# quasirandom/decoupled-kg

Measured on AMD Instinct MI355X. Metric: KG-evals/s (q=1, n_train=256, n_disc=1024, 16×128 MC) at 1/2/4/8 MI355X, higher is better.
Workload: dtype f64

## Files before the change

### decoupled-kg_amd/csrc/dkg_common.h

```cpp
#pragma once

#include <hip/hip_runtime.h>
#include <stdint.h>

#include <map>
#include <mutex>
#include <utility>

#include "dkg.h"

namespace dkg {

inline void raise_lds_limit(const void* kernel, size_t lds) {
  if (lds <= 65536) return;
  static std::mutex mu;
  static std::map<std::pair<const void*, int>, size_t> done;
  int dev = 0;
  (void)hipGetDevice(&dev);
  std::lock_guard<std::mutex> lock(mu);
  size_t& cur = done[{kernel, dev}];
  if (cur >= lds) return;
  if (hipFuncSetAttribute(kernel, hipFuncAttributeMaxDynamicSharedMemorySize, (int)lds) == hipSuccess) cur = lds;
}

// ... 195 lines not shown
__device__ __forceinline__ double norm_pdf(double c) { return 0.3989422804014327 * exp(-0.5 * c * c); }
__device__ __forceinline__ double norm_cdf(double c) { return 0.5 * erfc(-0.7071067811865476 * c); }

__device__ __forceinline__ double scaled_r2(const double* __restrict__ xa, const double* __restrict__ xb,
                                            const double* __restrict__ il, int d) {
  double acc = 0.0;
  for (int k = 0; k < d; ++k) {
    const double t = (xa[k] - xb[k]) * il[k];
    acc = fma(t, t, acc);
  }
  return acc;
}

template <int DM>
__device__ __forceinline__ double scaled_r2_dm(const double* __restrict__ xa, const double* __restrict__ xb,
                                               const double* __restrict__ il, int d) {
  double acc = 0.0;
#pragma unroll
  for (int k = 0; k < DM; ++k) {
    const int kk = min(k, d - 1);
    const double t = (xa[kk] - xb[kk]) * il[kk];
    acc = fma(t, (k < d) ? t : 0.0, acc);
  }
  return acc;
}

__host__ __device__ inline int dim_bucket(int d) { return d <= 2 ? 2 : d <= 4 ? 4 : d <= 8 ? 8 : 16; }

template <int CTRL>
__device__ __forceinline__ double dpp_f64(double v) {
  const int lo = __builtin_amdgcn_mov_dpp(__double2loint(v), CTRL, 0xF, 0xF, false);
  const int hi = __builtin_amdgcn_mov_dpp(__double2hiint(v), CTRL, 0xF, 0xF, false);
  return __hiloint2double(hi, lo);
}

template <int STEP>
__device__ __forceinline__ double partner_f64(double v) {
  if constexpr (STEP == 0) return dpp_f64<0xB1>(v);
  else if constexpr (STEP == 1) return dpp_f64<0x4E>(v);
  else if constexpr (STEP == 2) return dpp_f64<0x141>(v);
  else if constexpr (STEP == 3) return dpp_f64<0x140>(v);
  else return __shfl_xor(v, STEP == 4 ? 16 : 32);
}

#define DKG_BUTTERFLY(...)                         \
  {                                                \
    { constexpr int S_ = 0; __VA_ARGS__ }          \
    { constexpr int S_ = 1; __VA_ARGS__ }          \
    { constexpr int S_ = 2; __VA_ARGS__ }          \
    { constexpr int S_ = 3; __VA_ARGS__ }          \
    { constexpr int S_ = 4; __VA_ARGS__ }          \
    { constexpr int S_ = 5; __VA_ARGS__ }          \
  }

#define DKG_BUTTERFLY_ROW(...)                     \
  {                                                \
    { constexpr int S_ = 0; __VA_ARGS__ }          \
    { constexpr int S_ = 1; __VA_ARGS__ }          \
    { constexpr int S_ = 2; __VA_ARGS__ }          \
    { constexpr int S_ = 3; __VA_ARGS__ }          \
  }

__device__ __forceinline__ double fmin_raw(double a, double b) {
  double r;
  asm("v_min_f64 %0, %1, %2" : "=v"(r) : "v"(a), "v"(b));
  return r;
}
__device__ __forceinline__ double fmax_raw(double a, double b) {
  double r;
  asm("v_max_f64 %0, %1, %2" : "=v"(r) : "v"(a), "v"(b));
  return r;
}
__device__ __forceinline__ double keep_or_qnan(bool c, double v) {
  return __hiloint2double(c ? __double2hiint(v) : 0x7FF80000, __double2loint(v));
}

__device__ __forceinline__ double readlane_f64(double v, int l);

__device__ __forceinline__ double sgpr_f64(double v) {
  return __hiloint2double(__builtin_amdgcn_readfirstlane(__double2hiint(v)),
                          __builtin_amdgcn_readfirstlane(__double2loint(v)));
}


template <class Op>
__device__ __forceinline__ double combine_rows(double v, Op op) {
  const double r0 = readlane_f64(v, 0), r1 = readlane_f64(v, 16);
  const double r2 = readlane_f64(v, 32), r3 = readlane_f64(v, 48);
  return sgpr_f64(op(op(r0, r1), op(r2, r3)));
}

__device__ __forceinline__ int wave_min_i32(int v) {
  v = min(v, __builtin_amdgcn_mov_dpp(v, 0xB1, 0xF, 0xF, false));
  v = min(v, __builtin_amdgcn_mov_dpp(v, 0x4E, 0xF, 0xF, false));
  v = min(v, __builtin_amdgcn_mov_dpp(v, 0x141, 0xF, 0xF, false));
  v = min(v, __builtin_amdgcn_mov_dpp(v, 0x140, 0xF, 0xF, false));
  const int r0 = __builtin_amdgcn_readlane(v, 0), r1 = __builtin_amdgcn_readlane(v, 16);
  const int r2 = __builtin_amdgcn_readlane(v, 32), r3 = __builtin_amdgcn_readlane(v, 48);
  return min(min(r0, r1), min(r2, r3));
}

__device__ __forceinline__ double wave_sum(double v) {
  DKG_BUTTERFLY_ROW({ v = v + partner_f64<S_>(v); })
  return combine_rows(v, [](double a, double b) { return a + b; });
}

__device__ __forceinline__ double wave_max(double v) {
  DKG_BUTTERFLY_ROW({ v = fmax(v, partner_f64<S_>(v)); })
  return combine_rows(v, [](double a, double b) { return fmax(a, b); });
}

__device__ __forceinline__ uint64_t ballot(bool c) { return __builtin_amdgcn_ballot_w64(c); }

__device__ __forceinline__ bool uniform(bool c) { return __builtin_amdgcn_readfirstlane((int)c) != 0; }

__device__ __forceinline__ double readlane_f64(double v, int l) {
  const int lo = __builtin_amdgcn_readlane(__double2loint(v), l);
  const int hi = __builtin_amdgcn_readlane(__double2hiint(v), l);
  return __hiloint2double(hi, lo);
}

__device__ __forceinline__ double gather_f64(double v, int l) {
  const int lo = __builtin_amdgcn_ds_bpermute(l << 2, __double2loint(v));
  const int hi = __builtin_amdgcn_ds_bpermute(l << 2, __double2hiint(v));
  return __hiloint2double(hi, lo);
}

__device__ __forceinline__ int lanes_below(uint64_t mask) {
  return __builtin_amdgcn_mbcnt_hi((uint32_t)(mask >> 32), __builtin_amdgcn_mbcnt_lo((uint32_t)mask, 0));
}


__device__ __forceinline__ double psi(double c) {
  const const_dptr tab = psi_tab();
  const double x = fabs(c);
  const double x2 = x * x, x2l = fma(x, x, -x2);
  const double e = 0.3989422804014327 * exp_nonpos(-0.5 * x2, tab) * fma(-0.5, x2l, 1.0);
  double g;
  if (x < 4.0) {
    const double v = 0.25 * x;
    g = horner<9>(tab + PSI_OFF_PA, v) / horner<9>(tab + PSI_OFF_QA, v);
  } else {
    const double s = 1.0 / (x * x);
    const double u = (s - 0.000625) * 16.161616161616163;
    g = s * (horner<7>(tab + PSI_OFF_PB, u) / horner<7>(tab + PSI_OFF_QB, u));
  }
  const double r = e * g;
  return (c < 0.0) ? r + x : r;
}

__host__ __device__ inline int xcd_group_size(int nblk, int groups) { return 8 * groups * ((nblk + 7) / 8); }
__device__ __forceinline__ bool xcd_group(int L, int nblk, int groups, int& blk, int& member) {
  const int r = L >> 3;
  member = r % groups;
  blk = (r / groups) * 8 + (L & 7);
  return blk < nblk;
}

__host__ __device__ inline int block_order_size(int nbx, int nby, int m, int order) {
  if (order == 3) return 8 * ((nbx + 7) / 8) * nby * m;
  return order == 0 ? xcd_group_size(nbx * nby, m) : 8 * ((nbx * nby * m + 7) / 8);
}
__device__ __forceinline__ bool block_order(int L, int nbx, int nby, int m, int order, int& bx, int& by, int& oi) {
  if (order == 0) {
    int blk;
    if (!xcd_group(L, nbx * nby, m, blk, oi)) return false;
// ... 95 lines not shown
```

### decoupled-kg_amd/csrc/dkg_device.h

```cpp
#pragma once

#include <type_traits>

#include "dkg_common.h"
#include "dkg_kernels.h"
#include "dkg_walk.h"

namespace dkg {

__device__ __forceinline__ unsigned long long* kst_slot(int dst, const Plan* P, int kid) {
  if (dst != 1) return nullptr;
  const int wg = (blockIdx.z * gridDim.y + blockIdx.y) * gridDim.x + blockIdx.x;
  return (threadIdx.x == 0 && wg < KST_WG) ? P->kstamps + ((size_t)kid * KST_WG + wg) * 8 : nullptr;
}
#define KST_BEGIN(st)                                                  \
  do {                                                                 \
    if (st) {                                                          \
      (st)[0] = __builtin_amdgcn_s_memrealtime();                      \
      (st)[1] = __builtin_amdgcn_s_memtime();                          \
    }                                                                  \
  } while (0)
#define KST(st, k)                                                     \
  do {                                                                 \
    if (st) (st)[k] = __builtin_amdgcn_s_memtime();                    \
// ... 1065 lines not shown
          }
        }
        cnt += __popcll(mk[u]);
      }
    }
  }
}

__device__ __forceinline__ FwdEnv list_extremes(int cnt, int lane, const double* sb, const double* sa) {
  __builtin_amdgcn_fence(__ATOMIC_RELEASE, "wavefront");
  __builtin_amdgcn_wave_barrier();
  __builtin_amdgcn_fence(__ATOMIC_ACQUIRE, "wavefront");
  ExtAcc e;
  for (int q = 0; 64 * q < cnt; ++q) {
    const int i = lane + 64 * q;
    const bool live = i < cnt;
    const int ii = live ? i : 0;
    const double a = sa[ii], b = sb[ii];
    const bool l = live & ((b < e.bmin) | ((b == e.bmin) & (a > e.aLx)));
    e.bmin = l ? b : e.bmin;
    e.aLx = l ? a : e.aLx;
    const bool r = live & ((b > e.bmax) | ((b == e.bmax) & (a > e.aRx)));
    e.bmax = r ? b : e.bmax;
    e.aRx = r ? a : e.aRx;
    const bool tt = live & ((a > e.amax) | ((a == e.amax) & (b < e.bTx)));
    e.amax = tt ? a : e.amax;
    e.bTx = tt ? b : e.bTx;
  }
  return ext_reduce(e);
}

template <int MAXL, class Build>
__device__ __forceinline__ EdgeSum env_pair_stream_tail(const FwdEnv& f, int cnt, int nch, int nl, int lane,
                                                        double* sb, double* sa, int* si, double* vreg,
                                                        bool force_walk, int* nhull, Build&& build) {
  if (cnt > LIST_CAP_STREAM && !force_walk) cnt = refine_stream<MAXL>(f, nch, nl, lane, sb, sa, si, vreg, build);
  if (cnt >= 0 && cnt <= LIST_CAP_STREAM && !force_walk) {
    __builtin_amdgcn_fence(__ATOMIC_RELEASE, "wavefront");
    __builtin_amdgcn_wave_barrier();
    __builtin_amdgcn_fence(__ATOMIC_ACQUIRE, "wavefront");
    double cmax;
    EdgeSum kg;
    int h;
    if (cnt <= 128) kg = walk_small(cnt, lane, sb, sa, si, f.bL, f.aL, f.bT, &h, &cmax);
    else if (cnt <= 256) kg = walk_list<4>(cnt, lane, sb, sa, si, f.bL, f.aL, f.bT, &h, &cmax);
    else kg = walk_list<8>(cnt, lane, sb, sa, si, f.bL, f.aL, f.bT, &h, &cmax);
    if (uniform(cmax <= WALK_XGUARD)) {
      *nhull = h;
      return kg;
    }
  }
  return walk_stream<MAXL>(nch, nl, lane, f.bL, f.aL, f.bT, nhull, build);
}

template <int MAXL, class Build>
__device__ __forceinline__ EdgeSum env_pair_stream_edges(int nch, int nl, int lane, double* sb, double* sa, int* si,
                                                  double* vreg, bool force_walk, int* nhull, Build&& build) {
  const FwdEnv f = env_extremes_stream<MAXL>(nch, nl, lane, build);
  if (f.status == 1) {
    *nhull = 1;
    return EdgeSum{0.0, 0.0, 0.0, false};
  }
  const EnvChords ch = env_chords(f.bL, f.aL, f.bT, f.aT, f.bR, f.aR);
  int cnt = 0;
  for (int c = 0; c < nch; ++c) {
    double la[MAXL], lb[MAXL];
    build(c, la, lb);
    stream_keep<MAXL>(la, lb, c * 64 * MAXL, nl, ch, lane, sb, sa, si, cnt);
  }
  return env_pair_stream_tail<MAXL>(f, cnt, nch, nl, lane, sb, sa, si, vreg, force_walk, nhull, build);
}

template <int MAXL, class Build>
__device__ __forceinline__ double env_pair_stream(int nch, int nl, int lane, double* sb, double* sa, int* si,
                                                  double* vreg, bool force_walk, int* nhull, Build&& build) {
  return finish_edges(env_pair_stream_edges<MAXL>(nch, nl, lane, sb, sa, si, vreg, force_walk, nhull, build));
}

template <int M>
__device__ __forceinline__ void pair_coefs(const double* wrow, int m, bool full, int target, const double (&ysd)[M],
                                           const double (&ymu)[M], const double (&nz)[M], const double (&sv)[M],
                                           double (&w)[M], double (&wa)[M], double (&wb)[M], double& a_off,
                                           double& den) {
  a_off = 0.0;
  den = 0.0;
#pragma unroll
  for (int i = 0; i < M; ++i) {
    w[i] = (i < m) ? wrow[i] : 0.0;
    wa[i] = w[i] * ysd[i];
    a_off = fma(w[i], ymu[i], a_off);
    den = fma(w[i] * w[i], ysd[i] * ysd[i] * (sv[i] + nz[i]), den);
  }
  if (full) {
    const double inv_den = 1.0 / sqrt(den);
#pragma unroll
    for (int i = 0; i < M; ++i) wb[i] = w[i] * w[i] * ysd[i] * ysd[i] * inv_den;
  } else {
#pragma unroll
    for (int i = 0; i < M; ++i) {
      const double sd2 = ysd[i] * ysd[i];
      wb[i] = (i == target) ? w[i] * sd2 / sqrt(sd2 * (sv[i] + nz[i])) : 0.0;
    }
  }
}

__host__ __device__ inline int stage_len(int N) { return ((N + 127) / 128) * 128; }


constexpr int STAGE_FRONT = 8;

__host__ __device__ inline int stage_stride(int N, int rec) {
  const int slots = 64 * env_slots(N + 1) * rec;
  return (stage_len(N * rec) > slots ? stage_len(N * rec) : slots) + STAGE_FRONT;
}

struct EnvLds {
  int SLp;
  int LC;
  int NPS;
  int lmu;
  int lcv;
  int lw;
  int skg;
  int sbuf;
  int cbuf;
  int sif;
  int sidx;
  int qrow;
  int jrow;
  int sgv;
  int sgm;
  int sgw;
  int sx;
  int sil;
  int shD;
  int suw;
  int sscl;
  int shk;
  int total;
};

__host__ __device__ __forceinline__ EnvLds env_lds(int M, int m, int N, int SW, int S, int d, int NP, bool grad,
                                                   bool stream, bool grows) {
  EnvLds L;
  const int rec = cov_rec(M);
  L.SLp = stream ? 0 : stage_stride(N, rec);
  L.LC = list_cap(stream && !grad);
  L.NPS = stage_len(NP);
  L.lmu = STAGE_FRONT;
  L.lcv = L.lmu + L.SLp;
  L.lw = L.lcv + L.SLp;
  L.skg = L.lw + ((S * m + 1) & ~1);
  L.sbuf = L.skg + ((S + 1) & ~1);
  const int lists_end = L.sbuf + SW * 2 * L.LC;
  L.cbuf = L.sif = -1;
  L.sidx = L.qrow = L.jrow = L.sgv = L.sgm = L.sgw = L.sx = L.sil = L.shD = L.suw = L.sscl = L.shk = -1;
  if (!grad) {
    const int verts = SW * VREG, chunks = stream_staged(M) ? 4 * staged_chunk_len(rec) : 0;
    L.cbuf = lists_end;
    L.sif = L.cbuf + (!stream ? 0 : chunks > verts ? chunks : verts);
    L.total = L.sif + (SW * L.LC + 1) / 2;
    return L;
  }
  L.sidx = lists_end;
  L.sgv = L.sidx + (SW * ENV_CAP + 1) / 2;
  if (!grows) {
// ... 29 lines not shown
#define DKG_ENV_FWD_WPE 4
#endif
__host__ __device__ constexpr int env_waves_per_eu(int maxl, int m, bool grad, bool stream) {
  return (grad || stream || maxl > 17) ? 2 : (m >= 8 && maxl > 8) ? 3 : DKG_ENV_FWD_WPE;
}


template <int MAXL, int M, bool GRAD, bool STREAM, bool HO = false, bool MT = false, bool GROWS = false>
__device__ __forceinline__ void envelope_body(const Plan* __restrict__ P, int B, double* __restrict__ kg,
                                              double* __restrict__ pairs_out, int dst,
                                              const double* __restrict__ xnew, double* __restrict__ dkg,
                                              const double* __restrict__ mu_all, const double* __restrict__ cov_all,
                                              const double* __restrict__ var_all,
                                              const double* __restrict__ mux_all, const double* __restrict__ wts,
                                              const int* __restrict__ dupv, long long cov_stride, int bpad, int b,
                                              int g, int G, double* smem, unsigned long long* st,
                                              const Handoff* ho = nullptr, double* __restrict__ hout = nullptr,
                                              int tau = 0, int ntgt = 1, int target_mt = -1) {
  static_assert(!HO || (!GRAD && !STREAM), "the fused forward stages its lines (no gradient, no streaming)");
  static_assert(!GROWS || (GRAD && STREAM), "global rows: the streaming gradient envelope only");
  constexpr int NPP = 8;
  __shared__ double s_pp[DKG_MAX_OUTPUTS * NPP];
  __shared__ int s_kind[DKG_MAX_OUTPUTS];
  const int SW = blockDim.x >> 6;
  const int lane_k = threadIdx.x & 63;
  const int wave = __builtin_amdgcn_readfirstlane(threadIdx.x >> 6);
  const int m = P->m;
  const int N = P->N;
  const int NL = N + 1;
  const int S = P->S;
  const int target = MT ? target_mt : P->target;
  const bool full = target < 0;
  const size_t ib = MT ? (size_t)tau * B + b : (size_t)b, iw = MT ? (size_t)tau * bpad + b : (size_t)b;
  const size_t nitems = MT ? (size_t)ntgt * B : (size_t)B;
  static_assert(STREAM || MAXL == 2 || MAXL == 8 || MAXL == 17 || MAXL == 33, "slot bucket");
  KST_BEGIN(st);

  const double* mu_src[M];
  const double* cv_src[M];
#pragma unroll
  for (int i = 0; i < M; ++i) {
    mu_src[i] = mu_all;
    cv_src[i] = cov_all + (size_t)b * cov_stride;
  }

  constexpr int MP = cov_rec(M);
  const int d = P->d;
  const int NP = P->max_np;
  const EnvLds L = env_lds(M, m, N, SW, S, d, NP, GRAD, STREAM, GROWS);
  const int LC = L.LC, NPS = L.NPS;
  double* lmu = smem + L.lmu;
  double* lcv = smem + L.lcv;
  double* lw = smem + L.lw;
  double* skg = smem + L.skg;
  double* sbuf = smem + L.sbuf;
  const double* disc = GRAD ? P->disc : nullptr;
  const bool force_walk = __builtin_amdgcn_readfirstlane(P->debug_env) & 1;
  int* sidx = nullptr;
  double *qrow = nullptr, *jrow = nullptr, *sgv = nullptr, *sgm = nullptr, *sgw = nullptr, *sx = nullptr;
  double *sil = nullptr, *shD = nullptr, *suw = nullptr, *sscl = nullptr;
  int* shk = nullptr;
  if constexpr (GRAD) {
    double* at = sbuf;
    int at_off = L.sbuf;
    auto region = [&](int off) { at += off - at_off; at_off = off; return at; };
    sidx = reinterpret_cast<int*>(region(L.sidx));
    if constexpr (!GROWS) {
      qrow = region(L.qrow);
      jrow = region(L.jrow);
    }
    sgv = region(L.sgv);
    sgm = region(L.sgm);
    sgw = region(L.sgw);
    sx = region(L.sx);
    sil = region(L.sil);
    shD = region(L.shD);
    suw = region(L.suw);
    sscl = region(L.sscl);
    shk = reinterpret_cast<int*>(region(L.shk));
  }

  double pp[NPP] = {1.0, 0.0, 0.0, 0.0, 0.0, 0.0, 0.0, 0.0};
  double g_gm[M], g_il[M], g_x = 0.0;
  if (threadIdx.x < m) {
    const dkg_output* o = &P->o[threadIdx.x];
    pp[0] = o->y_std;
    pp[1] = o->y_mean;
    pp[2] = o->noise;
    pp[3] = o->outputscale;
    if constexpr (!HO) {
      pp[4] = var_all[(size_t)threadIdx.x * bpad + b];
      pp[5] = mux_all[(size_t)threadIdx.x * bpad + b];
      pp[6] = pp[5];
      pp[7] = pp[4];
    }
    if constexpr (GRAD) s_kind[threadIdx.x] = o->kernel;
  }
  const double* wsrc = wts;
  if constexpr (!STREAM) {
    dma_to_lds(mu_src[0], lmu, N * MP, wave, SW, lane_k);
    if constexpr (!HO) dma_to_lds(cv_src[0], lcv, N * MP, wave, SW, lane_k);
  }
  if constexpr (GRAD && !GROWS) {
#pragma unroll
    for (int i = 0; i < M; ++i) {
      if (i < m) {
        const int npi = pad16(P->o[i].n);
        const size_t mat = (size_t)P->bpad * npi;
        dma_to_lds(P->qxrm[i] + (size_t)b * npi, qrow + (size_t)i * NPS, npi, wave, SW, lane_k);
        for (int dd = 0; dd < d; ++dd)
          dma_to_lds(P->jq[i] + dd * mat + (size_t)b * npi, jrow + ((size_t)i * d + dd) * NPS, npi, wave, SW, lane_k);
      }
    }
  }
  for (int e = threadIdx.x; e < S * m; e += blockDim.x) lw[e] = wsrc[e];
  int dupk = DUP_NONE;
  if constexpr (!HO) dupk = dupv[b];
  double hA1 = 0.0;
  int hk1 = 0, hc1 = 0;
  constexpr bool HINT = !GRAD && !STREAM && !HO;
  if constexpr (HINT) {
    if (P->itop != nullptr) {
      const int jh = min(g * SW + wave, S - 1);
      hA1 = P->itop[jh];
      hk1 = P->itopk[2 * jh];
      hc1 = P->itopk[2 * jh + 1];
    }
  }
  if (threadIdx.x < m) {
#pragma unroll
    for (int q = 0; q < (HO ? 4 : NPP); ++q) s_pp[threadIdx.x * NPP + q] = pp[q];
  }
  if constexpr (HO) {
    handoff_wait(ho->cnt2 + (size_t)(b / ho->rb_rows) * HANDOFF_STRIDE, 1, ho->quota2, ho->err, 2);
    if (threadIdx.x < m) {
      s_pp[threadIdx.x * NPP + 4] = s_pp[threadIdx.x * NPP + 7] = var_all[(size_t)threadIdx.x * bpad + b];
      s_pp[threadIdx.x * NPP + 5] = s_pp[threadIdx.x * NPP + 6] = mux_all[(size_t)threadIdx.x * bpad + b];
    }
    dupk = dupv[b];
    dma_to_lds(cv_src[0], lcv, N * MP, wave, SW, lane_k);
  }
  if constexpr (GRAD) {
#pragma unroll
    for (int i = 0; i < M; ++i) {
      g_gm[i] = 0.0;
      g_il[i] = 0.0;
      if (i < m && threadIdx.x < d) {
        g_gm[i] = P->gmu[i][(size_t)threadIdx.x * P->bpad + b];
        g_il[i] = P->o[i].inv_lengthscale[threadIdx.x];
      }
    }
    if (threadIdx.x < d) g_x = xnew[(size_t)b * d + threadIdx.x];
  }
  const int SLd = STREAM ? 0 : stage_len(N * MP);
  const int pad_end = (64 * MAXL - 1) * MP;
  auto pad_lines = [&](int lo, int hi) {
    for (int e = lo + (int)threadIdx.x; e < hi; e += blockDim.x) {
      lmu[e] = __builtin_nan("");
      lcv[e] = __builtin_nan("");
    }
  };
  if constexpr (!STREAM) pad_lines(max(N * MP, SLd), pad_end);
  const int j0 = g * SW, j1 = min(S, j0 + SW);
  if (!GRAD) KST(st, 2);
  asm volatile("s_waitcnt vmcnt(0)" ::: "memory");
  __syncthreads();
  if constexpr (!STREAM) {
    if (SLd > N * MP) {
      pad_lines(N * MP, min(SLd, pad_end));
      __syncthreads();
    }
  }
  dupk = __builtin_amdgcn_readfirstlane(dupk);
  if (dupk != DUP_NONE) {
    if (threadIdx.x < m) {
      s_pp[threadIdx.x * NPP + 6] = mu_all[(size_t)dupk * MP + threadIdx.x];
      s_pp[threadIdx.x * NPP + 7] = cov_all[(size_t)b * cov_stride + (size_t)dupk * MP + threadIdx.x];
    }
    __syncthreads();
  }
  if constexpr (GRAD) {
    if (threadIdx.x < d) {
      sx[threadIdx.x] = g_x;
#pragma unroll
      for (int i = 0; i < M; ++i) {
        if (i < m) {
          sgm[i * DKG_MAX_DIM + threadIdx.x] = g_gm[i];
          sil[i * DKG_MAX_DIM + threadIdx.x] = g_il[i];
        }
      }
    }
    if constexpr (!GROWS) {
      bool tail = false;
#pragma unroll
      for (int i = 0; i < M; ++i) {
        if (i < m) {
          const int npi = pad16(P->o[i].n);
          if (npi < NP) {
            tail = true;
            for (int c = npi + (int)threadIdx.x; c < NP; c += blockDim.x) {
              qrow[(size_t)i * NPS + c] = 0.0;
              for (int dd = 0; dd < d; ++dd) jrow[((size_t)i * d + dd) * NPS + c] = 0.0;
            }
          }
        }
      }
      if (tail) __syncthreads();
    }
  }
  if (!GRAD) KST(st, 3);

  double* sb = sbuf + (size_t)wave * 2 * LC;
  double* sa = sb + LC;
  constexpr bool STG = STREAM && !GRAD && stream_staged(M);
  constexpr int CBL = STG ? staged_chunk_len(cov_rec(M)) : 0;
  double* cbuf = smem + L.cbuf;
  double* vreg = cbuf + (size_t)wave * VREG;
  int* sif = reinterpret_cast<int*>(smem + L.sif) + (size_t)wave * LC;
  int* si = nullptr;
  double* gw = nullptr;
  if constexpr (GRAD) {
    si = sidx + (size_t)wave * ENV_CAP;
    gw = sgw + wave * 64;
    for (int pidx = wave; pidx < m * d; pidx += SW) {
      const int i = pidx / d, dd = pidx % d;
      double acc = 0.0;
      if constexpr (GROWS) {
        const int npi = pad16(P->o[i].n);
        const double* qg = P->qxrm[i] + (size_t)b * npi;
        const double* jg = P->jq[i] + ((size_t)dd * bpad + b) * npi;
        for (int c = lane_k; c < NP; c += 64) {
          const int cc = min(c, npi - 1);
          const double jv = (c < npi) ? jg[cc] : 0.0, qv = (c < npi) ? qg[cc] : 0.0;
          acc = fma(jv, qv, acc);
        }
      } else {
        for (int c = lane_k; c < NP; c += 64) acc = fma(jrow[((size_t)i * d + dd) * NPS + c], qrow[(size_t)i * NPS + c], acc);
      }
      acc = wave_sum(acc);
      if (lane_k == 0) sgv[i * DKG_MAX_DIM + dd] = -2.0 * acc;
    }
    gw[lane_k] = 0.0;
    __syncthreads();
    KST(st, 2);
  }
  double sv[M], mx0[M], ysd[M], ymu[M], nz[M], os[M], l0m[M], l0v[M];
#pragma unroll
  for (int i = 0; i < M; ++i) {
    const bool live = i < m;
    ysd[i] = sgpr_f64(live ? s_pp[i * NPP + 0] : 1.0);
    ymu[i] = sgpr_f64(live ? s_pp[i * NPP + 1] : 0.0);
    nz[i] = sgpr_f64(live ? s_pp[i * NPP + 2] : 0.0);
    os[i] = sgpr_f64(live ? s_pp[i * NPP + 3] : 0.0);
    sv[i] = sgpr_f64(live ? s_pp[i * NPP + 4] : 0.0);
    mx0[i] = sgpr_f64(live ? s_pp[i * NPP + 5] : 0.0);
    l0m[i] = sgpr_f64(live ? s_pp[i * NPP + 6] : 0.0);
    l0v[i] = sgpr_f64(live ? s_pp[i * NPP + 7] : 0.0);
  }

  FwdEnv sf;
  int scnt = 0;
  if constexpr (STG) {
    constexpr int CS = STAGED_SLOTS, SCH = 64 * CS;
    const int lane = lane_k;
    const bool has = j0 + wave < j1;
    const int jj = has ? j0 + wave : j0;
    double w[M], wa[M], wb[M];
    double a_off, den;
    pair_coefs<M>(lw + jj * m, m, full, target, ysd, ymu, nz, sv, w, wa, wb, a_off, den);
#pragma unroll
    for (int i = 0; i < M; ++i) {
      wa[i] = sgpr_f64(wa[i]);
      wb[i] = sgpr_f64(wb[i]);
    }
    a_off = sgpr_f64(a_off);
    double bb0 = 0.0, a0 = a_off, wbt = 0.0;
#pragma unroll
    for (int i = 0; i < M; ++i) {
      bb0 = fma(wb[i], l0v[i], bb0);
      a0 = fma(wa[i], l0m[i], a0);
      wbt = (i == target) ? wb[i] : wbt;
    }
    const int nq = (NL + SCH - 1) / SCH;
    const double* cvb = cov_all + (size_t)b * cov_stride;
    auto stage = [&](int q) {
      constexpr int NP2 = MP / 2, GR = SCH / 64, NI = NP2 * GR;
      double* bm = cbuf + (size_t)(q & 1) * 2 * CBL;
      for (int ii = wave; ii < 2 * NI; ii += SW) {
        const int arr = ii / NI, rem = ii % NI, q2 = rem / GR, gi = rem % GR;
        const double* src = arr ? cvb : mu_all;
        const int rec = min(max(q * SCH - 1 + gi * 64 + lane_k, 0), N - 1);
        __builtin_amdgcn_global_load_lds(reinterpret_cast<const void*>(src + (size_t)rec * MP + 2 * q2),
                                         reinterpret_cast<__attribute__((address_space(3))) void*>(
                                             reinterpret_cast<uintptr_t>(bm + (size_t)arr * CBL +
                                                                         ((size_t)q2 * SCH + gi * 64) * 2)),
                                         16, 0, 0);
      }
    };
    auto build_staged = [&](int q, double (&la)[CS], double (&lb)[CS]) {
      const double* bm = cbuf + (size_t)(q & 1) * 2 * CBL;
      const double* mur = bm + lane * 2;
      const double* cvr = bm + CBL + lane * 2;
      const int kbase = q * SCH;
      auto adot = [&](const double* r, const double (&c)[M], double acc) __attribute__((always_inline)) {
#pragma unroll
        for (int q2 = 0; 2 * q2 < M; ++q2) {
          const double2 u = *reinterpret_cast<const double2*>(r + (size_t)q2 * SCH * 2);
          acc = fma(c[2 * q2], u.x, acc);
          if (2 * q2 + 1 < M) acc = fma(c[2 * q2 + 1], u.y, acc);
        }
        return acc;
      };
      const int tg = full ? 0 : target;
      const double* cvt = cvr + (size_t)(tg >> 1) * SCH * 2 + (tg & 1);
      if (full) {
#pragma unroll
        for (int t = 0; t < CS; ++t) {
          la[t] = adot(mur + 128 * t, wa, a_off);
          lb[t] = adot(cvr + 128 * t, wb, 0.0);
        }
      } else {
#pragma unroll
        for (int t = 0; t < CS; ++t) {
          la[t] = adot(mur + 128 * t, wa, a_off);
          lb[t] = fma(wbt, cvt[128 * t], 0.0);
        }
      }
#pragma unroll
      for (int t = 0; t < CS; ++t) {
        if (kbase + 64 * t + 63 > N) {
          const bool pad = kbase + lane + 64 * t > N;
          la[t] = pad ? -INFINITY : la[t];
// ... 2 lines not shown
      }
      if (q == 0) {
        la[0] = (lane == 0) ? a0 : la[0];
        lb[0] = (lane == 0) ? bb0 : lb[0];
      }
    };
    const int stride = (NL + SCH - 1) / SCH;
    {
      constexpr int NP2 = MP / 2, GR = SCH / 64, NI = NP2 * GR;
      for (int ii = wave; ii < 2 * NI; ii += SW) {
        const int arr = ii / NI, rem = ii % NI, q2 = rem / GR, gi = rem % GR;
        const double* src = arr ? cvb : mu_all;
        const int rec = min(max((gi * 64 + lane_k) * stride - 1, 0), N - 1);
        __builtin_amdgcn_global_load_lds(reinterpret_cast<const void*>(src + (size_t)rec * MP + 2 * q2),
                                         reinterpret_cast<__attribute__((address_space(3))) void*>(
                                             reinterpret_cast<uintptr_t>(cbuf + (size_t)arr * CBL +
                                                                         ((size_t)q2 * SCH + gi * 64) * 2)),
                                         16, 0, 0);
      }
    }
    asm volatile("s_waitcnt vmcnt(0)" ::: "memory");
    __syncthreads();
    ChainChords<SH_NC> cc;
    bool chain_ok = false;
    if (has && !(__builtin_amdgcn_readfirstlane(P->debug_env) & 8)) {
      double la[CS], lb[CS];
      build_staged(0, la, lb);
      ExtAcc es;
      ext_fold<CS>(la, lb, 0, SCH, lane, es);
      const FwdEnv fs = ext_reduce(es);
      double* vb = cbuf + 2 * (size_t)CBL + (size_t)wave * VREG;
      double* va = vb + VCAP;
      if (fs.status == 0) {
        if (lane == 0) {
          vb[0] = fs.bL; va[0] = fs.aL;
          vb[1] = fs.bT; va[1] = fs.aT;
          vb[2] = fs.bR; va[2] = fs.aR;
        }
        __builtin_amdgcn_fence(__ATOMIC_RELEASE, "wavefront");
        __builtin_amdgcn_wave_barrier();
        __builtin_amdgcn_fence(__ATOMIC_ACQUIRE, "wavefront");
        int nv = 3, tpos = 1;
        auto sample = [&](int, double (&xa)[CS], double (&xb)[CS]) {
#pragma unroll
          for (int t = 0; t < CS; ++t) { xa[t] = la[t]; xb[t] = lb[t]; }
        };
        if (qh_extend<CS, 3>(1, SCH, lane, vb, va, nv, tpos, sample) > 0 && SH_ROUNDS > 1)
          qh_extend<CS, 5>(1, SCH, lane, vb, va, nv, tpos, sample);
        double bm = 0.0;
#pragma unroll
        for (int i = 0; i < M; ++i)
          bm = fma(fabs(wb[i]), sqrt(fmax(sv[i], 0.0) * fmax(os[i], 0.0)) + 1e-8 * fabs(os[i]), bm);
        cc = chain_chords<SH_NC>(vb, va, nv, 2.0 * bm * (1.0 + 1e-6));
        chain_ok = true;
      }
    }
    __syncthreads();
#ifdef DKG_STG_STAMPS
    if (st) st[4] = __builtin_amdgcn_s_memtime();
#endif
    stage(0);
    for (int q = 0; q < nq; ++q) {
      asm volatile("s_waitcnt vmcnt(0)" ::: "memory");
      __syncthreads();
      if (q + 1 < nq) stage(q + 1);
      if (chain_ok) {
        double la[CS], lb[CS];
        build_staged(q, la, lb);
        chain_keep<CS, SH_NC>(la, lb, q * SCH, NL, cc, lane, sb, sa, sif, scnt);
      }
    }
    __syncthreads();
#ifdef DKG_STG_STAMPS
    if (st) st[5] = __builtin_amdgcn_s_memtime();
#endif
    if (!chain_ok) scnt = LIST_CAP_STREAM + 1;
    sf.status = 0;
  }

  if (const int j = j0 + wave; j < j1) {
    const int lane = lane_k;
    double w[M], wa[M], wb[M];
    double a_off, den;
    pair_coefs<M>(lw + j * m, m, full, target, ysd, ymu, nz, sv, w, wa, wb, a_off, den);
#pragma unroll
    for (int i = 0; i < M; ++i) {
      w[i] = sgpr_f64(w[i]);
      wa[i] = sgpr_f64(wa[i]);
      wb[i] = sgpr_f64(wb[i]);
    }
    a_off = sgpr_f64(a_off);
    den = sgpr_f64(den);
    double bb0 = 0.0;
#pragma unroll
    for (int i = 0; i < M; ++i) bb0 = fma(wb[i], l0v[i], bb0);
    auto build_chunk = [&](int c, double (&la)[MAXL], double (&lb)[MAXL]) {
      const int kbase = c * 64 * MAXL;
      const size_t rowoff = (size_t)b * cov_stride;
      const int nmax = max(N, 1) - 1;
#pragma unroll
      for (int t = 0; t < MAXL; ++t) {
        const int k = kbase + lane + 64 * t;
        const int idx = min(max(k - 1, 0), nmax);
        double a = a_off, bb = 0.0;
#pragma unroll
        for (int i = 0; i < M; ++i) {
          if (i < m) {
            a = fma(wa[i], mu_all[(size_t)idx * MP + i], a);
            if (full || i == target) bb = fma(wb[i], cov_all[rowoff + (size_t)idx * MP + i], bb);
          }
        }
        la[t] = a;
        lb[t] = bb;
        if (kbase + 64 * t + 63 > N) {
          const bool pad = k > N;
          la[t] = pad ? -INFINITY : la[t];
          lb[t] = pad ? bb0 : lb[t];
        }
      }
      if (c == 0) {
        double a = a_off;
#pragma unroll
        for (int i = 0; i < M; ++i) a = fma(wa[i], l0m[i], a);
        la[0] = (lane == 0) ? a : la[0];
        lb[0] = (lane == 0) ? bb0 : lb[0];
      }
    };
    const int nch = (NL + 64 * MAXL - 1) / (64 * MAXL);
    auto build_lines = [&](double (&la)[MAXL], double (&lb)[MAXL]) {
      const double* mur = lmu + (lane - 1) * MP;
      const double* cvr = lcv + (lane - 1) * MP;
      auto rec_dot = [&](const double* r, const double (&c)[M], double acc) __attribute__((always_inline)) {
        if constexpr (MP == 1) {
          acc = fma(c[0], r[0], acc);
        } else {
#pragma unroll
          for (int q = 0; 2 * q < M; ++q) {
            const double2 u = *reinterpret_cast<const double2*>(r + 2 * q);
            acc = fma(c[2 * q], u.x, acc);
            if (2 * q + 1 < M) acc = fma(c[2 * q + 1], u.y, acc);
          }
        }
        return acc;
      };
      if (full) {
#pragma unroll
        for (int t = 0; t < MAXL; ++t) {
          la[t] = rec_dot(mur + 64 * MP * t, wa, a_off);
          lb[t] = rec_dot(cvr + 64 * MP * t, wb, 0.0);
        }
      } else {
        const double* cvt = cvr + target;
        double wbt = 0.0;
#pragma unroll
        for (int i = 0; i < M; ++i) wbt = (i == target) ? wb[i] : wbt;
#pragma unroll
        for (int t = 0; t < MAXL; ++t) {
          la[t] = rec_dot(mur + 64 * MP * t, wa, a_off);
          lb[t] = wbt * cvt[64 * MP * t];
        }
      }
      {
        double a = a_off, bb = 0.0;
#pragma unroll
        for (int i = 0; i < M; ++i) {
          a = fma(wa[i], l0m[i], a);
          bb = fma(wb[i], l0v[i], bb);
        }
        la[0] = (lane == 0) ? a : la[0];
        lb[0] = (lane == 0) ? bb : lb[0];
      }
    };

    double kgj;
    int hn = 1;
    if constexpr (GRAD) {
      EnvFilter f;
      if constexpr (STREAM) {
        f = envelope_filter_stream<MAXL, true>(nch, lane, sb, sa, si, build_chunk);
      } else {
        double la[MAXL], lb[MAXL];
        build_lines(la, lb);
        bool flat = false;
        if (!force_walk) {
          FwdEnv fe;
          env_top<MAXL>(la, lb, fe);
          if (env_flat<MAXL>(la, lb, fe)) {
            const double a0l = readlane_f64(la[0], 0);
            int ct = 0;
#pragma unroll
            for (int t = 0; t < MAXL; ++t) ct += __popcll(ballot(la[t] == fe.aT));
            flat = !(a0l == fe.aT) || ct == 1;
          }
        }
        if (flat)
          f.status = 3;
        else
          f = envelope_filter<MAXL, true>(la, lb, lane, sb, sa, si);
      }
      if (force_walk && f.status == 0) f.status = 2;
      if (j == j0 + wave) KST(st, 3);
      double Vden = den;
      if (!full) {
        const double sd2 = ysd[target] * ysd[target];
        Vden = sd2 * (sv[target] + nz[target]);
      }
      if (lane == 0) {
        for (int dd = 0; dd < d; ++dd) {
          double ga0 = 0.0, gvs = 0.0;
#pragma unroll
          for (int i = 0; i < M; ++i) {
            if (i < m) {
              ga0 = fma(wa[i], sgm[i * DKG_MAX_DIM + dd], ga0);
              const double cv = full ? w[i] * w[i] * ysd[i] * ysd[i] : ((i == target) ? ysd[i] * ysd[i] : 0.0);
              gvs = fma(cv, sgv[i * DKG_MAX_DIM + dd], gvs);
            }
          }
          gw[16 + dd] = ga0;
          gw[32 + dd] = gvs / (2.0 * Vden);
        }
      }
      double sumDb = 0.0;
      int* hk = shk + wave * HCAP;
      double* scl = sscl + wave * ENV_CAP;
      double* hD = shD + wave * HCAP;
      double* uw = suw + (size_t)wave * NP;
      int nh = 0;
      auto flush = [&]() __attribute__((always_inline)) {
        __builtin_amdgcn_fence(__ATOMIC_RELEASE, "wavefront");
        __builtin_amdgcn_wave_barrier();
        __builtin_amdgcn_fence(__ATOMIC_ACQUIRE, "wavefront");
        for (int h0 = 0; h0 < nh; h0 += 64) {
          const bool act = h0 + lane < nh;
          const int k = act ? hk[h0 + lane] : 1;
          const double Dw = act ? hD[h0 + lane] : 0.0;
          const double* z = disc + (size_t)(k - 1) * d;
          double hc[M];
#pragma unroll
          for (int i = 0; i < M; ++i) {
            hc[i] = 0.0;
            if (i < m && wb[i] != 0.0) {
              double r2 = 0.0;
              for (int dd = 0; dd < d; ++dd) {
                const double t = (sx[dd] - z[dd]) * sil[i * DKG_MAX_DIM + dd];
                r2 = fma(t, t, r2);
              }
              hc[i] = Dw * wb[i] * os[i] * kernel_dprofile(__builtin_amdgcn_readfirstlane(s_kind[i]), r2);
            }
          }
          for (int dd = 0; dd < d; ++dd) {
            const double t = sx[dd] - z[dd];
// ... 110 lines not shown
            kR = (lb[t] == f.bR && la[t] == f.aR) ? k : kR;
            ct += __popcll(ballot(la[t] == f.aT));
          }
        };
        if constexpr (STREAM) {
          for (int c = nch - 1; c >= 0; --c) {
            double la[MAXL], lb[MAXL];
            build_chunk(c, la, lb);
            scan(la, lb, c * 64 * MAXL);
          }
        } else {
          double la[MAXL], lb[MAXL];
          build_lines(la, lb);
          scan(la, lb, 0);
        }
        DKG_BUTTERFLY({
          const int st = S_ == 0 ? 1 : S_ == 1 ? 2 : S_ == 2 ? 4 : S_ == 3 ? 8 : S_ == 4 ? 16 : 32;
          kL = min(kL, __shfl_xor(kL, st));
          kT = min(kT, __shfl_xor(kT, st));
          kR = min(kR, __shfl_xor(kR, st));
        })
        f.kL = __builtin_amdgcn_readfirstlane(kL);
        f.kT = __builtin_amdgcn_readfirstlane(kT);
        f.kR = __builtin_amdgcn_readfirstlane(kR);
        f.cntT = ct;
      }
      if (f.status == 1 || f.status == 3) {
        kgj = 0.0;
      } else {
        if (f.status == 0) {
          const HullGrad hg = envelope_hull_grad(f, lane, sb, sa, si, scl, hk, hD, N);
          kgj = hg.kg;
          sumDb = hg.sumDb;
          nh = hg.nq;
          f.cntT = hg.cntT;
          if (lane == 0) {
            for (int dd = 0; dd < d; ++dd) {
              double gvs = 0.0;
#pragma unroll
              for (int i = 0; i < M; ++i)
                if (i < m) gvs = fma(wb[i], sgv[i * DKG_MAX_DIM + dd], gvs);
              gw[dd] += hg.Dw0 * gvs + hg.Pw0 * gw[16 + dd];
            }
          }
        } else if constexpr (STREAM) {
          kgj = envelope_walk_stream<MAXL>(nch, NL, lane, f, build_chunk, visit, f.kL);
        } else {
          auto rebuild = [&](int, double (&la)[MAXL], double (&lb)[MAXL]) { build_lines(la, lb); };
          kgj = envelope_walk_stream<MAXL>(1, NL, lane, f, rebuild, visit, f.kL);
        }
        if (j == j0 + wave) KST(st, 4);
        if (nh > 0) flush();
        if (j == j0 + wave) KST(st, 5);
        double a0 = a_off;
#pragma unroll
        for (int i = 0; i < M; ++i) a0 = fma(wa[i], l0m[i], a0);
        const double tfac = (a0 == f.aT) ? 1.0 / (double)f.cntT : 0.0;
        if (lane == 0)
          for (int dd = 0; dd < d; ++dd) gw[48 + dd] += gw[dd] - sumDb * gw[32 + dd] - tfac * gw[16 + dd];
      }
      if (lane == 0)
        for (int dd = 0; dd < d; ++dd) gw[dd] = 0.0;
    } else if constexpr (STG) {
      sf = (scnt <= LIST_CAP_STREAM) ? list_extremes(scnt, lane, sb, sa) : env_extremes_stream<MAXL>(nch, NL, lane,
                                                                                                     build_chunk);
#ifdef DKG_STG_STAMPS
      if (lane == 0) P->hull_pairs[iw * S + j] = scnt;
#endif
      if (sf.status == 1) {
        kgj = 0.0;
        hn = 1;
      } else {
        kgj = finish_edges(env_pair_stream_tail<MAXL>(sf, scnt, nch, NL, lane, sb, sa, sif, vreg, force_walk, &hn,
                                                      build_chunk));
      }
    } else if constexpr (STREAM) {
      kgj = env_pair_stream<MAXL>(nch, NL, lane, sb, sa, sif, vreg, force_walk, &hn, build_chunk);
    } else {
      unsigned long long* pst = (dst == 2 && (size_t)b * S + j < 2 * KST_WG)
                                    ? P->kstamps + ((size_t)b * S + j) * 8 : nullptr;
      const bool flat_ok = pairs_out == nullptr && !force_walk;
      TopHint hint{false, 0.0, 0.0};
      if (HINT && flat_ok && P->itop != nullptr) {
        double a0 = a_off, b0 = 0.0;
#pragma unroll
        for (int i = 0; i < M; ++i) {
          a0 = fma(wa[i], l0m[i], a0);
          b0 = fma(wb[i], l0v[i], b0);
        }
        const double A1 = hA1;
        const int k1 = hk1, c1 = hc1;
        if (a0 > A1) {
          hint = TopHint{true, a0, b0};
        } else if (a0 < A1 && c1 == 1) {
          const double* r = lcv + (size_t)(k1 - 1) * MP;
          double bk = 0.0;
          if (full) {
            if constexpr (MP == 1) {
              bk = fma(wb[0], r[0], bk);
            } else {
#pragma unroll
              for (int q = 0; 2 * q < M; ++q) {
                const double2 u = *reinterpret_cast<const double2*>(r + 2 * q);
                bk = fma(wb[2 * q], u.x, bk);
                if (2 * q + 1 < M) bk = fma(wb[2 * q + 1], u.y, bk);
              }
            }
          } else {
            double wbt = 0.0;
#pragma unroll
            for (int i = 0; i < M; ++i) wbt = (i == target) ? wb[i] : wbt;
            bk = wbt * r[target];
          }
          hint = TopHint{true, A1, bk};
        }
      }
      auto rebuild = [&](double (&la)[MAXL], double (&lb)[MAXL]) { build_lines(la, lb); };
      kgj = env_pair_regs<MAXL>(rebuild, NL, lane, sb, sa, sif, force_walk, &hn, nullptr, pst, flat_ok, hint);
    }
    if (pairs_out != nullptr && lane == 0) {
      pairs_out[ib * S + j] = kgj;
#ifdef DKG_STG_STAMPS
      if constexpr (!GRAD && !STG) P->hull_pairs[iw * S + j] = hn;
#else
      if constexpr (!GRAD) P->hull_pairs[iw * S + j] = hn;
#endif
    }
    if (lane == 0) skg[j - j0] = kgj;
  }

#ifndef DKG_STG_STAMPS
  if (!GRAD) KST(st, 4);
#endif
  __syncthreads();
#ifndef DKG_STG_STAMPS
  if (!GRAD) KST(st, 5);
#endif
  {
    const int ng = (S + 7) >> 3;
    const int grp = j0 >> 3;
    const int gpairs = min(8, S - 8 * grp);
    const int gwgs = (gpairs + SW - 1) / SW;
    const size_t prow = iw * (S + ng);
    int* tk = P->tickets + iw * (ng + 1);
    __shared__ int s_last;
    const int dg = GRAD ? d : 0;
    double gsum = 0.0;
    const int gi = (int)threadIdx.x - 1;
    if (gwgs == 1) {
      if (threadIdx.x == 0)
        for (int q = 0; q < j1 - j0; ++q) gsum += skg[q];
      if (GRAD && gi >= 0 && gi < dg)
        for (int q = 0; q < j1 - j0; ++q) gsum += sgw[q * 64 + 48 + gi];
    } else {
      if (threadIdx.x == 0)
        for (int q = 0; q < j1 - j0; ++q) __hip_atomic_store(&P->wg_part[prow + j0 + q], skg[q], __ATOMIC_RELAXED,
                                                             __HIP_MEMORY_SCOPE_AGENT);
      if (GRAD && gi >= 0 && gi < dg)
        for (int q = 0; q < j1 - j0; ++q)
          __hip_atomic_store(&P->wg_gpart[(prow + j0 + q) * dg + gi], sgw[q * 64 + 48 + gi], __ATOMIC_RELAXED,
                             __HIP_MEMORY_SCOPE_AGENT);
      asm volatile("s_waitcnt vmcnt(0)" ::: "memory");
      __syncthreads();
      if (threadIdx.x == 0)
        s_last = __hip_atomic_fetch_add(&tk[grp], 1, __ATOMIC_RELAXED, __HIP_MEMORY_SCOPE_AGENT) == gwgs - 1;
      __syncthreads();
      if (s_last) {
        if (threadIdx.x == 0)
          for (int q = 8 * grp; q < 8 * grp + gpairs; ++q)
            gsum += __hip_atomic_load(&P->wg_part[prow + q], __ATOMIC_RELAXED, __HIP_MEMORY_SCOPE_AGENT);
        if (GRAD && gi >= 0 && gi < dg)
          for (int q = 8 * grp; q < 8 * grp + gpairs; ++q)
// ... 261 lines not shown
```

Before: 17.30 million.

## Precompute per-pair line coefficients once per workgroup in wave 0 via LDS rows

For the plain (non-grad, non-stream, non-handoff) kernel path, wave 0 loads output parameters and weight rows directly into registers. It computes each wave's pair coefficients (wa, wb, a_off and the line-0 intercept and slope) once and writes them as a row in each wave's survivor buffer. Every wave then reads its row instead of staging weights and per-output parameters through LDS and recomputing them. The itop hints are also loaded through the constant address space, and FP contraction is disabled in pair_coefs, which changes rounding slightly. This shortens per-pair setup and prologue work, at the cost of more serial work on wave 0 and added register pressure.

Result: faster. 17.59 million (median of 6 runs) (+1.7%).

```diff
diff --git a/decoupled-kg_amd/csrc/dkg_common.h b/decoupled-kg_amd/csrc/dkg_common.h
--- a/decoupled-kg_amd/csrc/dkg_common.h
+++ b/decoupled-kg_amd/csrc/dkg_common.h
@@ -301,6 +301,11 @@
                           __builtin_amdgcn_readfirstlane(__double2loint(v)));
 }
 
+__device__ __forceinline__ double pin_sgpr_f64(double v) {
+  int hi = __double2hiint(v), lo = __double2loint(v);
+  asm volatile("" : "+s"(hi), "+s"(lo));
+  return __hiloint2double(hi, lo);
+}
 
 template <class Op>
 __device__ __forceinline__ double combine_rows(double v, Op op) {
diff --git a/decoupled-kg_amd/csrc/dkg_device.h b/decoupled-kg_amd/csrc/dkg_device.h
--- a/decoupled-kg_amd/csrc/dkg_device.h
+++ b/decoupled-kg_amd/csrc/dkg_device.h
@@ -1171,6 +1171,7 @@
                                            const double (&ymu)[M], const double (&nz)[M], const double (&sv)[M],
                                            double (&w)[M], double (&wa)[M], double (&wb)[M], double& a_off,
                                            double& den) {
+#pragma clang fp contract(off)
   a_off = 0.0;
   den = 0.0;
 #pragma unroll
@@ -1366,19 +1367,26 @@
 
   double pp[NPP] = {1.0, 0.0, 0.0, 0.0, 0.0, 0.0, 0.0, 0.0};
   double g_gm[M], g_il[M], g_x = 0.0;
+  const int j0 = g * SW, j1 = min(S, j0 + SW);
+  constexpr bool COEF1 = !GRAD && !STREAM && !HO;
+  constexpr int ENV_MAX_WAVES = 512 / 64;
+  constexpr int NPC = 2 * M + 3;
+  static_assert(NPC <= 2 * ENV_CAP, "a pair's coefficient row fits its wave's survivor list");
   if (threadIdx.x < m) {
-    const dkg_output* o = &P->o[threadIdx.x];
-    pp[0] = o->y_std;
-    pp[1] = o->y_mean;
-    pp[2] = o->noise;
-    pp[3] = o->outputscale;
-    if constexpr (!HO) {
+    if constexpr (!COEF1) {
+      const dkg_output* o = &P->o[threadIdx.x];
+      pp[0] = o->y_std;
+      pp[1] = o->y_mean;
+      pp[2] = o->noise;
+      pp[3] = o->outputscale;
+    }
+    if constexpr (!HO && !COEF1) {
       pp[4] = var_all[(size_t)threadIdx.x * bpad + b];
       pp[5] = mux_all[(size_t)threadIdx.x * bpad + b];
       pp[6] = pp[5];
       pp[7] = pp[4];
     }
-    if constexpr (GRAD) s_kind[threadIdx.x] = o->kernel;
+    if constexpr (GRAD) s_kind[threadIdx.x] = P->o[threadIdx.x].kernel;
   }
   const double* wsrc = wts;
   if constexpr (!STREAM) {
@@ -1397,7 +1405,42 @@
       }
     }
   }
-  for (int e = threadIdx.x; e < S * m; e += blockDim.x) lw[e] = wsrc[e];
+  if constexpr (!COEF1)
+    for (int e = threadIdx.x; e < S * m; e += blockDim.x) lw[e] = wsrc[e];
+  double c_w[M], c_ysd[M], c_ymu[M], c_nz[M], c_sv[M], c_mx[M];
+  if constexpr (COEF1) {
+    if (wave == 0) {
+#pragma unroll
+      for (int i = 0; i < M; ++i) {
+        const bool live = i < m;
+        const int ic = min(i, m - 1);
+        const dkg_output* o = &P->o[ic];
+        const double ysd_i = o->y_std, ymu_i = o->y_mean, nz_i = o->noise;
+        const double sv_i = var_all[(size_t)ic * bpad + b], mx_i = mux_all[(size_t)ic * bpad + b];
+        c_ysd[i] = live ? ysd_i : 1.0;
+        c_ymu[i] = live ? ymu_i : 0.0;
+        c_nz[i] = live ? nz_i : 0.0;
+        c_sv[i] = live ? sv_i : 0.0;
+        c_mx[i] = live ? mx_i : 0.0;
+        c_w[i] = 0.0;
+      }
+      double wr[ENV_MAX_WAVES][M];
+#pragma unroll
+      for (int p = 0; p < ENV_MAX_WAVES; ++p) {
+        const double* wrow = wts + (size_t)min(j0 + p, j1 - 1) * m;
+#pragma unroll
+        for (int i = 0; i < M; ++i) wr[p][i] = wrow[min(i, m - 1)];
+      }
+#pragma unroll
+      for (int p = 0; p < ENV_MAX_WAVES; ++p) {
+#pragma unroll
+        for (int i = 0; i < M; ++i) {
+          const double v = pin_sgpr_f64(wr[p][i]);
+          c_w[i] = (lane_k >= p) ? v : c_w[i];
+        }
+      }
+    }
+  }
   int dupk = DUP_NONE;
   if constexpr (!HO) dupk = dupv[b];
   double hA1 = 0.0;
@@ -1406,12 +1449,14 @@
   if constexpr (HINT) {
     if (P->itop != nullptr) {
       const int jh = min(g * SW + wave, S - 1);
-      hA1 = P->itop[jh];
-      hk1 = P->itopk[2 * jh];
-      hc1 = P->itopk[2 * jh + 1];
-    }
-  }
-  if (threadIdx.x < m) {
+      const auto* itop_c = (const __attribute__((address_space(4))) double*)P->itop;
+      const auto* itopk_c = (const __attribute__((address_space(4))) int*)P->itopk;
+      hA1 = itop_c[jh];
+      hk1 = itopk_c[2 * jh];
+      hc1 = itopk_c[2 * jh + 1];
+    }
+  }
+  if (!COEF1 && threadIdx.x < m) {
 #pragma unroll
     for (int q = 0; q < (HO ? 4 : NPP); ++q) s_pp[threadIdx.x * NPP + q] = pp[q];
   }
@@ -1445,7 +1490,30 @@
     }
   };
   if constexpr (!STREAM) pad_lines(max(N * MP, SLd), pad_end);
-  const int j0 = g * SW, j1 = min(S, j0 + SW);
+  if constexpr (COEF1) {
+    if (wave == 0) {
+      double w[M], wa[M], wb[M];
+      double a_off, den;
+      pair_coefs<M>(c_w, m, full, target, c_ysd, c_ymu, c_nz, c_sv, w, wa, wb, a_off, den);
+      double a0 = a_off, b0 = 0.0;
+#pragma unroll
+      for (int i = 0; i < M; ++i) {
+        a0 = fma(wa[i], c_mx[i], a0);
+        b0 = fma(wb[i], c_sv[i], b0);
+      }
+      if (lane_k < j1 - j0) {
+        double* row = sbuf + (size_t)lane_k * 2 * LC;
+#pragma unroll
+        for (int i = 0; i < M; ++i) {
+          row[i] = wa[i];
+          row[M + i] = wb[i];
+        }
+        row[2 * M] = a_off;
+        row[2 * M + 1] = a0;
+        row[2 * M + 2] = b0;
+      }
+    }
+  }
   if (!GRAD) KST(st, 2);
   asm volatile("s_waitcnt vmcnt(0)" ::: "memory");
   __syncthreads();
@@ -1532,6 +1600,15 @@
 #pragma unroll
   for (int i = 0; i < M; ++i) {
     const bool live = i < m;
+    if constexpr (COEF1) {
+      ysd[i] = 1.0;
+      ymu[i] = nz[i] = os[i] = sv[i] = mx0[i] = l0m[i] = l0v[i] = 0.0;
+      if (dupk != DUP_NONE) {
+        l0m[i] = sgpr_f64(live ? s_pp[i * NPP + 6] : 0.0);
+        l0v[i] = sgpr_f64(live ? s_pp[i * NPP + 7] : 0.0);
+      }
+      continue;
+    }
     ysd[i] = sgpr_f64(live ? s_pp[i * NPP + 0] : 1.0);
     ymu[i] = sgpr_f64(live ? s_pp[i * NPP + 1] : 0.0);
     nz[i] = sgpr_f64(live ? s_pp[i * NPP + 2] : 0.0);
@@ -1700,7 +1777,22 @@
     const int lane = lane_k;
     double w[M], wa[M], wb[M];
     double a_off, den;
-    pair_coefs<M>(lw + j * m, m, full, target, ysd, ymu, nz, sv, w, wa, wb, a_off, den);
+    double a0l = 0.0, b0l = 0.0;
+    if constexpr (COEF1) {
+      const double* row = sb;
+#pragma unroll
+      for (int i = 0; i < M; ++i) {
+        w[i] = 0.0;
+        wa[i] = row[i];
+        wb[i] = row[M + i];
+      }
+      a_off = row[2 * M];
+      den = 0.0;
+      a0l = row[2 * M + 1];
+      b0l = row[2 * M + 2];
+    } else {
+      pair_coefs<M>(lw + j * m, m, full, target, ysd, ymu, nz, sv, w, wa, wb, a_off, den);
+    }
 #pragma unroll
     for (int i = 0; i < M; ++i) {
       w[i] = sgpr_f64(w[i]);
@@ -1709,6 +1801,20 @@
     }
     a_off = sgpr_f64(a_off);
     den = sgpr_f64(den);
+    auto line0 = [&](double& a, double& bb) __attribute__((always_inline)) {
+      a = a_off;
+      bb = 0.0;
+#pragma unroll
+      for (int i = 0; i < M; ++i) {
+        a = fma(wa[i], l0m[i], a);
+        bb = fma(wb[i], l0v[i], bb);
+      }
+    };
+    if constexpr (COEF1) {
+      if (dupk != DUP_NONE) line0(a0l, b0l);
+      a0l = sgpr_f64(a0l);
+      b0l = sgpr_f64(b0l);
+    }
     double bb0 = 0.0;
 #pragma unroll
     for (int i = 0; i < M; ++i) bb0 = fma(wb[i], l0v[i], bb0);
@@ -1779,12 +1885,8 @@
         }
       }
       {
-        double a = a_off, bb = 0.0;
-#pragma unroll
-        for (int i = 0; i < M; ++i) {
-          a = fma(wa[i], l0m[i], a);
-          bb = fma(wb[i], l0v[i], bb);
-        }
+        double a = a0l, bb = b0l;
+        if constexpr (!COEF1) line0(a, bb);
         la[0] = (lane == 0) ? a : la[0];
         lb[0] = (lane == 0) ? bb : lb[0];
       }
@@ -2061,12 +2163,8 @@
       const bool flat_ok = pairs_out == nullptr && !force_walk;
       TopHint hint{false, 0.0, 0.0};
       if (HINT && flat_ok && P->itop != nullptr) {
-        double a0 = a_off, b0 = 0.0;
-#pragma unroll
-        for (int i = 0; i < M; ++i) {
-          a0 = fma(wa[i], l0m[i], a0);
-          b0 = fma(wb[i], l0v[i], b0);
-        }
+        double a0 = a0l, b0 = b0l;
+        if constexpr (!COEF1) line0(a0, b0);
         const double A1 = hA1;
         const int k1 = hk1, c1 = hc1;
         if (a0 > A1) {
```
